# OpenVisualCloud/SVT-VP9

Measured on AMD Instinct MI355X. Metric: hot-path frames/sec (+ Mpixels/sec): block-level DSP path (picture analysis + ME + inter prediction from reconstructed references + DCT/quant/recon + deblock + reference padding), 3840x2160p60 yuv420p enc-mode 8; no mode decision, no entropy coding -- not encoded frames, higher is better.
Workload: dtype u8

## Files before the change

svt-vp9_amd/csrc/encdec.hip:

```cpp
#include <hip/hip_runtime.h>
#include <stdlib.h>
#include <string.h>
#include "svt_ctx.h"
#include "encdec_core.h"

#define ED_MAX_PICS 32
#define ED_MAX_SETS 8

struct svt_encdec_work {
    int           max_pics, width, height, n_sb, sb_cols, mi_rows, mi_cols;
    size_t        cap_per_pic;
    svt_tq_block *d_blocks;
    void         *last_hb;
    uint32_t     *d_pos;
    uint16_t     *d_eob;
    int32_t      *d_counts;
    int32_t      *d_totals, *d_bases;
    int32_t      *d_off_cnt;
    int32_t      *d_status;
    int32_t      *d_intra_sync;
    svt_quant_tables *d_qtabs;
    int16_t      *d_iscan;
    svt_encdec_stage_hook hook;
    void         *hook_user;
// ... 346 lines not shown
        if (svt_ctx_stage(ctx, sizeof qt, &h, &d)) return svt_set_error(SVT_HIP_ERR_NO_RESOURCES, "encdec: descriptor buffers");
        memcpy(h, qt, sizeof qt);
        HIP_TRY(hipMemcpyAsync(w->d_qtabs, h, sizeof qt, hipMemcpyHostToDevice, ctx->stream));
        svt_ctx_stage_commit(ctx);
    }
#define ED_STAGE(k) do { if (w->hook) w->hook(w->hook_user, (k)); } while (0)
    ED_STAGE(SVT_ENCDEC_STAGE_MC);
    int32_t rc = svt_hip_inter_pred_batch_device(ctx, n_pics, mcp);
    if (rc) return rc;
    ED_STAGE(SVT_ENCDEC_STAGE_LISTS);
    const int nwg = n_pics * hb.n_sb;
    hipLaunchKernelGGL(svt_tq_count_kernel, dim3(nwg), dim3(64), 0, ctx->stream, dB, w->d_counts, w->d_status);
    hipLaunchKernelGGL(svt_scan_sb_kernel, dim3(4 * n_pics), dim3(256), 0, ctx->stream, w->d_counts, hb.n_sb, w->d_totals);
    hipLaunchKernelGGL(svt_scan_pic_kernel, dim3(1), dim3(64), 0, ctx->stream, (const int32_t *)w->d_totals, n_pics, w->d_bases, w->d_off_cnt);
    hipLaunchKernelGGL(svt_tq_emit_kernel, dim3(nwg), dim3(64), 0, ctx->stream, dB, (const int32_t *)w->d_counts, (const int32_t *)w->d_bases, (svt_tq_block *)nullptr, w->d_pos);
    HIP_TRY(hipGetLastError());
    if (!w->last_hb) w->last_hb = malloc(sizeof hb);
    if (w->last_hb) memcpy(w->last_hb, &hb, sizeof hb);
    ED_STAGE(SVT_ENCDEC_STAGE_TQ);
    int32_t cap[4];
    for (int s = 0; s < 4; s++) cap[s] = (int32_t)((size_t)n_pics * width * height * 3 / 2 / (size_t)(16 << (2 * s)));
    rc = svt_tq_launch_device_lists(ctx, (const uint8_t *)src_lo, (const uint8_t *)pred_lo, recon_set, n_sets, nullptr, cap, w->d_off_cnt, w->d_qtabs, w->d_iscan,
                                    (int16_t *)q_lo, (int16_t *)dq_lo, w->d_eob, nullptr, w->d_pos, &dB->pic[0].g, (int)sizeof(ed_pic_dev), dB->iscan_off, hb.sb_cols);
    if (rc) return rc;
    ED_STAGE(SVT_ENCDEC_STAGE_SKIP);
    {
        const size_t map_bytes = (size_t)(width / 4) * (height / 4) * 3 / 2 * sizeof(uint16_t);
        uintptr_t    low = map_bytes;
        for (int i = 0; i < n_pics; i++) low |= (uintptr_t)pics[i].d_eob_map;
        if (!(low & 15))
            hipLaunchKernelGGL(svt_eob_map_clear_kernel, dim3(64, n_pics), dim3(256), 0, ctx->stream, dB, (int)(map_bytes / 16));
        else
            for (int i = 0; i < n_pics; i++) HIP_TRY(hipMemsetAsync(pics[i].d_eob_map, 0, map_bytes, ctx->stream));
    }
    for (int i = 0; i < n_pics; i++)
        if (pics[i].has_intra) {
            if (!flags->do_recon) return svt_set_error(SVT_HIP_ERR_BAD_PARAMETER, "encdec: intra blocks need the reconstruction (do_recon)");
            rc = svt_intra_launch(ctx, &pics[i], width, height, mi_stride, w->d_qtabs, w->d_iscan, hb.iscan_off, w->d_intra_sync, w->d_status, 1);
            if (rc) return rc;
        }
    {
        const int total_cap = (int)(w->cap_per_pic * (size_t)n_pics);
        int       g = (total_cap + 255) / 256;
        if (g > ctx->cu_count * 8) g = ctx->cu_count * 8;
        hipLaunchKernelGGL(svt_tq_skip_kernel, dim3(g), dim3(256), 0, ctx->stream, dB, (const int32_t *)w->d_off_cnt, (const uint32_t *)w->d_pos, (const uint16_t *)w->d_eob);
        hipLaunchKernelGGL(svt_skip_update_kernel, dim3((n_pics * hb.mi_rows * hb.mi_cols + 255) / 256), dim3(256), 0, ctx->stream, dB);
        HIP_TRY(hipGetLastError());
    }
    ED_STAGE(SVT_ENCDEC_STAGE_LF);
    if (flags->apply_loop_filter) {
        hipLaunchKernelGGL(svt_lf_mask_kernel, dim3(nwg), dim3(64), 0, ctx->stream, dB, w->d_status);
        HIP_TRY(hipGetLastError());
        rc = svt_hip_lf_batch_device(ctx, n_pics, rec, lfm, lfm_stride, thr, mi_rows_a, mi_cols_a, 0);
        if (rc) return rc;
    }
    ED_STAGE(SVT_ENCDEC_STAGE_PAD);
    if (flags->pad_reference && n_rec_pad) {
        rc = svt_hip_ref_pad_batch_device(ctx, n_rec_pad, rec_pad, pad_x, pad_y);
        if (rc) return rc;
    }
    ED_STAGE(SVT_ENCDEC_STAGE_END);
    return SVT_HIP_OK;
}

extern "C" int32_t svt_hip_encdec_intra_device(svt_hip_ctx *ctx, svt_encdec_work *w, const svt_encdec_picture *pic, int32_t width, int32_t height, int32_t mi_stride,
                                               int32_t q_index, const svt_encdec_flags *flags, const svt_lf_thresh *thr, int32_t pad_x, int32_t pad_y) {
    if (!ctx || !w || !pic || !flags || width != w->width || height != w->height || mi_stride < (width >> 3))
        return svt_set_error(SVT_HIP_ERR_BAD_PARAMETER, "encdec_intra: bad argument");
    if (!flags->do_recon) return svt_set_error(SVT_HIP_ERR_BAD_PARAMETER, "encdec_intra: intra prediction needs the reconstruction (do_recon)");
    if (flags->apply_loop_filter && !thr) return svt_set_error(SVT_HIP_ERR_BAD_PARAMETER, "encdec_intra: loop filter without thresholds");
    const svt_encdec_picture &p = *pic;
    if (!p.d_lf_mi || !p.src.y || !p.src.u || !p.src.v || !p.recon.y || !p.recon.u || !p.recon.v || !p.d_qcoeff || !p.d_eob_map || !p.d_nz ||
        (flags->apply_loop_filter && !p.d_lfm))
        return svt_set_error(SVT_HIP_ERR_BAD_PARAMETER, "encdec_intra: null picture field");
    if (((uintptr_t)p.d_qcoeff | (uintptr_t)p.d_dqcoeff) & 15) return svt_set_error(SVT_HIP_ERR_BAD_PARAMETER, "encdec_intra: coefficient arrays must be 16-byte aligned");
    if (p.recon.y_stride > 65535 || ((p.src.y_stride | p.src.uv_stride | p.recon.y_stride | p.recon.uv_stride) & 3) ||
        (((uintptr_t)p.src.y | (uintptr_t)p.src.u | (uintptr_t)p.src.v | (uintptr_t)p.recon.y | (uintptr_t)p.recon.u | (uintptr_t)p.recon.v) & 3) ||
        (p.pred.y && (((uintptr_t)p.pred.y | (uintptr_t)p.pred.u | (uintptr_t)p.pred.v | (uintptr_t)p.pred.y_stride | (uintptr_t)p.pred.uv_stride) & 3)))
        return svt_set_error(SVT_HIP_ERR_BAD_PARAMETER, "encdec_intra: planes and strides must be 4-byte aligned");
    if (p.pred.y && (!p.pred.u || !p.pred.v)) return svt_set_error(SVT_HIP_ERR_BAD_PARAMETER, "encdec_intra: prediction planes");
    HIP_TRY(hipSetDevice(ctx->device));
    ed_batch_dev hb;
    memset(&hb, 0, sizeof hb);
    fill_dims(hb, 1, width, height, mi_stride);
    const uint32_t *offs = nullptr;
    (void)svt_hip_vp9_iscan_tables(&offs, nullptr);
    hb.pic[0].lf_mi = p.d_lf_mi; hb.pic[0].nz = p.d_nz; hb.pic[0].eob_map = p.d_eob_map; hb.pic[0].lfm = p.d_lfm;
    const ed_batch_dev *dB = nullptr;
    if (stage_batch(ctx, hb, &dB)) return svt_set_error(SVT_HIP_ERR_NO_RESOURCES, "encdec_intra: descriptor buffers");
    {
        svt_quant_tables qt[2];
        if (svt_hip_quant_tables_for_qindex(q_index, qt) != SVT_HIP_OK) return svt_set_error(SVT_HIP_ERR_BAD_PARAMETER, "encdec_intra: q index");
        void *h = nullptr, *d = nullptr;
        if (svt_ctx_stage(ctx, sizeof qt, &h, &d)) return svt_set_error(SVT_HIP_ERR_NO_RESOURCES, "encdec_intra: descriptor buffers");
        memcpy(h, qt, sizeof qt);
        HIP_TRY(hipMemcpyAsync(w->d_qtabs, h, sizeof qt, hipMemcpyHostToDevice, ctx->stream));
        svt_ctx_stage_commit(ctx);
    }
    ED_STAGE(SVT_ENCDEC_STAGE_TQ);
    HIP_TRY(hipMemsetAsync(p.d_eob_map, 0, (size_t)(width / 4) * (height / 4) * 3 / 2 * sizeof(uint16_t), ctx->stream));
    HIP_TRY(hipMemsetAsync(p.d_nz, 0, (size_t)mi_stride * hb.mi_rows, ctx->stream));
    int32_t rc = svt_intra_launch(ctx, pic, width, height, mi_stride, w->d_qtabs, w->d_iscan, offs, w->d_intra_sync, w->d_status, 0);
    if (rc) return rc;
    ED_STAGE(SVT_ENCDEC_STAGE_SKIP);
    hipLaunchKernelGGL(svt_skip_update_kernel, dim3((hb.mi_rows * hb.mi_cols + 255) / 256), dim3(256), 0, ctx->stream, dB);
    HIP_TRY(hipGetLastError());
    ED_STAGE(SVT_ENCDEC_STAGE_LF);
    svt_yuv_planes rec = p.recon;
    rec.width = width; rec.height = height;
    if (flags->apply_loop_filter) {
        hipLaunchKernelGGL(svt_lf_mask_kernel, dim3(hb.n_sb), dim3(64), 0, ctx->stream, dB, w->d_status);
        HIP_TRY(hipGetLastError());
        const svt_lf_mask *lfm = p.d_lfm;
        const int32_t      lfm_stride = hb.sb_cols, mr = hb.mi_rows, mc = hb.mi_cols;
        rc = svt_hip_lf_batch_device(ctx, 1, &rec, &lfm, &lfm_stride, thr, &mr, &mc, 0);
        if (rc) return rc;
    }
    ED_STAGE(SVT_ENCDEC_STAGE_PAD);
    if (flags->pad_reference && !p.no_pad) {
        rc = svt_hip_ref_pad_batch_device(ctx, 1, &rec, pad_x, pad_y);
        if (rc) return rc;
    }
    ED_STAGE(SVT_ENCDEC_STAGE_END);
    return SVT_HIP_OK;
}

extern "C" int32_t svt_hip_md_intra_default_device(svt_hip_ctx *ctx, int32_t width, int32_t height, int32_t filter_level, svt_lf_mode_info *d_lf_mi, int32_t mi_stride) {
    if (!ctx || !d_lf_mi || width < 8 || height < 8 || (width & 7) || (height & 7) || mi_stride < (width >> 3))
        return svt_set_error(SVT_HIP_ERR_BAD_PARAMETER, "md_intra_default: bad argument");
    HIP_TRY(hipSetDevice(ctx->device));
    return svt_md_intra_default_launch(ctx, d_lf_mi, mi_stride, height >> 3, width >> 3, filter_level);
}

extern "C" void svt_hip_encdec_work_set_stage_hook(svt_encdec_work *w, svt_encdec_stage_hook hook, void *user) {
    if (!w) return;
    w->hook = hook;
    w->hook_user = user;
}

extern "C" int32_t svt_hip_encdec_work_status(svt_hip_ctx *ctx, svt_encdec_work *w, int32_t counts[8]) {
    if (!ctx || !w) return svt_set_error(SVT_HIP_ERR_BAD_PARAMETER, "encdec_status: null");
    HIP_TRY(hipSetDevice(ctx->device));
    int32_t h[9];
    HIP_TRY(hipMemcpyAsync(h, w->d_off_cnt, sizeof h, hipMemcpyDeviceToHost, ctx->stream));
    HIP_TRY(hipStreamSynchronize(ctx->stream));
    if (counts) memcpy(counts, h, 8 * sizeof(int32_t));
    if (h[8]) {
        HIP_TRY(hipMemsetAsync(w->d_status, 0, sizeof(int32_t), ctx->stream));
        return svt_set_error(SVT_HIP_ERR_BAD_PARAMETER, "encdec: malformed mode-info grid (block outside the picture, misaligned, or transform larger than its block)");
    }
    return SVT_HIP_OK;
}

extern "C" int32_t svt_hip_encdec_work_download(svt_hip_ctx *ctx, svt_encdec_work *w, svt_tq_block *blocks, uint32_t *pos, uint16_t *eob, int32_t capacity) {
    int32_t c[8];
    const int32_t rc = svt_hip_encdec_work_status(ctx, w, c);
    if (rc) return rc;
    const int32_t total = c[3] + c[7];
    if (total > capacity) return svt_set_error(SVT_HIP_ERR_NO_RESOURCES, "encdec_download: capacity");
    if (total > 0) {
        if (blocks) {
            if (!w->last_hb) return svt_set_error(SVT_HIP_ERR_BAD_PARAMETER, "encdec_download: no batch yet");
            if (!w->d_blocks && hipMalloc((void **)&w->d_blocks, w->cap_per_pic * (size_t)w->max_pics * sizeof(svt_tq_block)) != hipSuccess) {
                w->d_blocks = nullptr;
                return svt_set_error(SVT_HIP_ERR_NO_RESOURCES, "encdec_download: device memory");
            }
            const ed_batch_dev *dB = nullptr;
            if (stage_batch(ctx, *(const ed_batch_dev *)w->last_hb, &dB)) return svt_set_error(SVT_HIP_ERR_NO_RESOURCES, "encdec_download: descriptor buffers");
            hipLaunchKernelGGL(svt_tq_expand_kernel, dim3((total + 255) / 256), dim3(256), 0, ctx->stream, dB, (const int32_t *)w->d_off_cnt, (const uint32_t *)w->d_pos, w->d_blocks);
            HIP_TRY(hipGetLastError());
            HIP_TRY(hipMemcpyAsync(blocks, w->d_blocks, (size_t)total * sizeof(svt_tq_block), hipMemcpyDeviceToHost, ctx->stream));
        }
        if (pos) HIP_TRY(hipMemcpyAsync(pos, w->d_pos, (size_t)total * sizeof(uint32_t), hipMemcpyDeviceToHost, ctx->stream));
        if (eob) HIP_TRY(hipMemcpyAsync(eob, w->d_eob, (size_t)total * sizeof(uint16_t), hipMemcpyDeviceToHost, ctx->stream));
        HIP_TRY(hipStreamSynchronize(ctx->stream));
    }
    return total;
}

extern "C" int32_t svt_hip_md_default_batch_device(svt_hip_ctx *ctx, int32_t n_pics, const svt_me_pu_result *const *d_results, int32_t width, int32_t height,
                                                   uint32_t lambda, int32_t filter_level, svt_mc_mode_info *const *d_mc_mi, svt_lf_mode_info *const *d_lf_mi,
                                                   int32_t mi_stride) {
    if (!ctx || n_pics < 1 || !d_results || !d_mc_mi || !d_lf_mi || width < 8 || height < 8 || (width & 7) || (height & 7) || mi_stride < (width >> 3))
        return svt_set_error(SVT_HIP_ERR_BAD_PARAMETER, "md_default: bad argument");
    HIP_TRY(hipSetDevice(ctx->device));
    for (int first = 0; first < n_pics; first += ED_MAX_PICS) {
        const int n = n_pics - first < ED_MAX_PICS ? n_pics - first : ED_MAX_PICS;
        ed_batch_dev hb;
        memset(&hb, 0, sizeof hb);
        fill_dims(hb, n, width, height, mi_stride);
        hb.lambda = lambda; hb.filter_level = filter_level;
        for (int i = 0; i < n; i++) {
            if (!d_results[first + i] || !d_mc_mi[first + i] || !d_lf_mi[first + i]) return svt_set_error(SVT_HIP_ERR_BAD_PARAMETER, "md_default: null picture");
            hb.pic[i].res = d_results[first + i]; hb.pic[i].mc_mi = d_mc_mi[first + i]; hb.pic[i].lf_mi = d_lf_mi[first + i];
        }
        const ed_batch_dev *dB = nullptr;
        if (stage_batch(ctx, hb, &dB)) return svt_set_error(SVT_HIP_ERR_NO_RESOURCES, "md_default: descriptor buffers");
        hipLaunchKernelGGL(svt_md_default_kernel, dim3(n * hb.n_sb), dim3(64), 0, ctx->stream, dB);
        HIP_TRY(hipGetLastError());
    }
    return SVT_HIP_OK;
}

extern "C" int32_t svt_hip_lf_build_masks_device(svt_hip_ctx *ctx, int32_t n_pics, const svt_lf_mode_info *const *d_lf_mi, int32_t mi_stride, int32_t mi_rows,
                                                 int32_t mi_cols, svt_lf_mask *const *d_lfm) {
    if (!ctx || n_pics < 1 || !d_lf_mi || !d_lfm || mi_rows < 1 || mi_cols < 1 || mi_stride < mi_cols) return svt_set_error(SVT_HIP_ERR_BAD_PARAMETER, "lf_masks: bad argument");
    HIP_TRY(hipSetDevice(ctx->device));
    for (int first = 0; first < n_pics; first += ED_MAX_PICS) {
        const int n = n_pics - first < ED_MAX_PICS ? n_pics - first : ED_MAX_PICS;
        ed_batch_dev hb;
        memset(&hb, 0, sizeof hb);
        fill_dims(hb, n, mi_cols * 8, mi_rows * 8, mi_stride);
        for (int i = 0; i < n; i++) {
            if (!d_lf_mi[first + i] || !d_lfm[first + i]) return svt_set_error(SVT_HIP_ERR_BAD_PARAMETER, "lf_masks: null picture");
            hb.pic[i].lf_mi = (svt_lf_mode_info *)d_lf_mi[first + i]; hb.pic[i].lfm = d_lfm[first + i];
        }
        const ed_batch_dev *dB = nullptr;
        if (stage_batch(ctx, hb, &dB)) return svt_set_error(SVT_HIP_ERR_NO_RESOURCES, "lf_masks: descriptor buffers");
        hipLaunchKernelGGL(svt_lf_mask_kernel, dim3(n * hb.n_sb), dim3(64), 0, ctx->stream, dB, (int32_t *)nullptr);
        HIP_TRY(hipGetLastError());
    }
    return SVT_HIP_OK;
}
```

svt-vp9_amd/csrc/intra_kernel.hip:

```cpp
#include <hip/hip_runtime.h>
#include "tq_core.h"
#include "encdec_core.h"
#include "intra_pred.h"
#include <stdlib.h>

namespace {

struct intra_pic_dev {
    const uint8_t *src[3];
    uint8_t       *pred[3];
    uint8_t       *rec[3];
    int32_t        src_stride[2], pred_stride[2], rec_stride[2];
    const svt_lf_mode_info *mi;
    int32_t        mi_stride, mi_rows, mi_cols, sb_cols, sb_rows, width, height;
    const svt_quant_tables *qtabs;
    const int16_t *iscan;
    uint32_t       iscan_off[16];
    int16_t       *qcoeff, *dqcoeff;
    uint16_t      *eob_map;
    uint8_t       *nz;
    int32_t       *sync;
    int32_t       *status;
    int32_t        mixed;
};

#ifdef INTRA_FENCES
#define INTRA_WT false
#define INTRA_LD(p) (*(p))
#else
#define INTRA_WT true
#define INTRA_LD(p) __hip_atomic_load((p), __ATOMIC_RELAXED, __HIP_MEMORY_SCOPE_AGENT)
#endif
#ifdef INTRA_PROF
__device__ unsigned long long g_intra_fine[8];
#define IPF(k) do { if (lane == 0) { const unsigned long long n_ = __builtin_amdgcn_s_memtime(); atomicAdd(&g_intra_fine[k], n_ - ipf_t); ipf_t = n_; } } while (0)
#else
#define IPF(k) ((void)0)
#endif
template <int N>
__device__ __forceinline__ int intra_block(const intra_pic_dev &P, int plane, int x0, int y0, int mode, int sb, int32_t *tile, uint8_t *edge, int have_right = 0) {
    const int lane = (int)threadIdx.x, c = plane ? 1 : 0;
    const int rs = P.rec_stride[c];
    uint8_t  *rp = P.rec[plane];
    const int have_left = x0 > 0, have_top = y0 > 0;
    const bool active = lane < N;
    const int  i = lane % N;
#ifdef INTRA_PROF
    unsigned long long ipf_t = __builtin_amdgcn_s_memtime();
#endif
    uint32_t   srow[N / 4], prow[N / 4];
    constexpr uintptr_t AM = N >= 16 ? 15 : N - 1;
    {
        const uint8_t *sp = P.src[plane] + (size_t)(y0 + i) * P.src_stride[c] + x0;
        _Pragma("unroll") for (int q = 0; q < N / 4; q++) srow[q] = 0u;
        if (active) row_load<N>(sp, ((uintptr_t)sp & AM) == 0, srow);
    }
    {
        const int j = lane & 31;
        if (lane < 32) {
            if (j < N) edge[32 - (j + 1)] = have_left ? INTRA_LD(&rp[(size_t)(y0 + j) * rs + x0 - 1]) : (uint8_t)129;
        } else {
            if (j < N) {
                const uint8_t a = have_top ? INTRA_LD(&rp[(size_t)(y0 - 1) * rs + x0 + j]) : (uint8_t)127;
                edge[32 + 1 + j] = a;
                if (N == 4 && have_right) edge[32 + 1 + N + j] = have_top ? INTRA_LD(&rp[(size_t)(y0 - 1) * rs + x0 + N + j]) : (uint8_t)127;
                else if (j == N - 1) { _Pragma("unroll") for (int q = 0; q < N; q++) edge[32 + 1 + N + q] = a; }
            }
        }
        if (lane == 0) edge[32] = have_top ? (have_left ? INTRA_LD(&rp[(size_t)(y0 - 1) * rs + x0 - 1]) : (uint8_t)129) : (uint8_t)127;
    }
    __syncthreads();
    IPF(0);
    intra_pred_row<N>(edge, mode, i, have_left, have_top, prow);
    {
        if (active && P.pred[plane]) {
            uint8_t *pp = P.pred[plane] + (size_t)(y0 + i) * P.pred_stride[c] + x0;
            row_store<N>(pp, ((uintptr_t)pp & AM) == 0, prow);
        }
    }
    IPF(1);
    svt_tq_block k;
    k.src_off = k.pred_off = 0;
    k.recon_off = (uint32_t)y0 * (uint32_t)rs + (uint32_t)x0;
    k.coeff_off = (uint32_t)sb * SVT_SB_COEFFS + (plane == 0 ? 0u : plane == 1 ? 4096u : 5120u) + svt_zorder4((x0 & (plane ? 31 : 63)) >> 2, (y0 & (plane ? 31 : 63)) >> 2) * 16u;
    k.tx_size = (uint8_t)txcfg<N>::size;
    k.tx_type = (uint8_t)((plane == 0 && N < 32) ? intra_tx_type(mode) : 0);
    k.iscan_off = P.iscan_off[k.tx_size * 4 + k.tx_type];
    k.src_stride = k.pred_stride = 0; k.recon_stride = (uint16_t)rs;
    k.qtab = (uint8_t)c; k.do_recon = 1; k.partial32 = 0; k.pad_[0] = 0;
    const int pw4 = (plane ? P.width >> 1 : P.width) >> 2, w4 = P.width >> 2, h4 = P.height >> 2;
    const int eo = plane == 0 ? 0 : w4 * h4 + (plane == 2 ? (w4 >> 1) * (h4 >> 1) : 0);
    int32_t *t = tile + (lane / N) * (N * (N + 1));
    const int eob = tq_block_body<N, false, false, INTRA_WT>(k, active, i, t, srow, prow, P.qtabs, P.iscan, P.qcoeff, P.dqcoeff,
                                                   P.eob_map + eo + (y0 >> 2) * pw4 + (x0 >> 2), nullptr, nullptr, nullptr, nullptr, nullptr, rp);
    IPF(2);
    __builtin_amdgcn_fence(__ATOMIC_SEQ_CST, "workgroup");
    __syncthreads();
    IPF(3);
    return __builtin_amdgcn_readfirstlane(eob);
}

#ifndef INTRA_WAVES_PER_EU
#define INTRA_WAVES_PER_EU 4
#endif
#ifdef INTRA_NUM_VGPR
__attribute__((amdgpu_num_vgpr(INTRA_NUM_VGPR)))
#endif
__global__ __launch_bounds__(64) __attribute__((amdgpu_waves_per_eu(INTRA_WAVES_PER_EU, INTRA_WAVES_PER_EU))) void svt_intra_kernel(const intra_pic_dev P) {
    __shared__ int32_t tile[2 * 32 * 33];
    __shared__ uint8_t edge[128];
    __shared__ int32_t s_ticket;
    const int lane = (int)threadIdx.x, c_cols = (P.width + 15) >> 4, c_rows = (P.height + 15) >> 4, n_cell = c_cols * c_rows;
    const int n_diag = c_rows + c_cols - 1;
    __builtin_amdgcn_s_setprio(3);
#ifdef INTRA_PROF
  unsigned long long pf[5] = {0, 0, 0, 0, 0}, pf_n = 0;
#endif
  for (;;) {
    __syncthreads();
    if (lane == 0) s_ticket = atomicAdd(&P.sync[0], 1);
    __syncthreads();
#ifdef INTRA_PROF
    if (s_ticket >= 3 * n_cell) { if (lane == 0 && blockIdx.x == 0) printf("[intra-fine] refs %llu predict %llu tq %llu drain %llu (summed over all workgroups so far)\n", g_intra_fine[0], g_intra_fine[1], g_intra_fine[2], g_intra_fine[3]);
      if (lane == 0 && blockIdx.x < 2) printf("[intra-prof] wg %d cells %llu: ticket+map %llu wait %llu work %llu drain %llu publish %llu (100 MHz ticks)\n", (int)blockIdx.x, pf_n, pf[0], pf[1], pf[2], pf[3], pf[4]); break; }
    unsigned long long pt0 = __builtin_amdgcn_s_memtime();
#else
    if (s_ticket >= 3 * n_cell) break;
#endif
    const int ticket = s_ticket, plane = ticket % 3;
    const int n = ticket / 3, m = c_rows < c_cols ? c_rows : c_cols, M = c_rows < c_cols ? c_cols : c_rows;
    int lo = 0, hi = n_diag;
    auto count = [&](int d) -> int {
        const int a = d < m ? d : m;
        int       t = a * (a + 1) / 2;
        if (d > m) { const int fl = (d < M ? d : M) - m; t += fl * m; }
        if (d > M) { const int k = d - M; t += k * m - k * (k + 1) / 2; }
        return t;
    };
    while (hi - lo > 1) { const int mid = (lo + hi) >> 1; if (count(mid) <= n) lo = mid; else hi = mid; }
    const int d = lo, r_lo = d - (c_cols - 1) > 0 ? d - (c_cols - 1) : 0;
    const int cr = r_lo + (n - count(d)), cc = d - cr;
    const int cell = cr * c_cols + cc;
    int32_t  *done = P.sync + 2 + plane * n_cell;
    const int  br = cr & ~1, bc = cc & ~1;
    const int  ub_r = br * 2, ub_c = bc * 2;
    const svt_lf_mode_info b0 = P.mi[ub_r * P.mi_stride + ub_c];
    const bool big = b0.sb_type == 9 && !(b0.is_inter && P.mixed) && ub_r + 4 <= P.mi_rows && ub_c + 4 <= P.mi_cols;
    if (big && !(cr == br && cc == bc + 1)) continue;
    const int ur0 = cr * 2, uc0 = cc * 2;
#ifdef INTRA_PROF
    unsigned long long pt1 = __builtin_amdgcn_s_memtime();
#endif
    if (lane == 0) {
        const int wl_r = big ? br + 1 : cr, wl_c = (big ? bc : cc) - 1;
        const int wa_r = (big ? br : cr) - 1, wa_c = big ? bc + 1 : cc;
        if (wl_c >= 0) while (__hip_atomic_load(&done[wl_r * c_cols + wl_c], __ATOMIC_RELAXED, __HIP_MEMORY_SCOPE_AGENT) == 0) __builtin_amdgcn_s_sleep(2);
        if (wa_r >= 0) while (__hip_atomic_load(&done[wa_r * c_cols + wa_c], __ATOMIC_RELAXED, __HIP_MEMORY_SCOPE_AGENT) == 0) __builtin_amdgcn_s_sleep(2);
    }
    __syncthreads();
#ifdef INTRA_FENCES
    __builtin_amdgcn_fence(__ATOMIC_ACQUIRE, "agent");
#endif
#ifdef INTRA_PROF
    unsigned long long pt2 = __builtin_amdgcn_s_memtime();
#endif
    const int nu = big ? 1 : 4, u_r = big ? ub_r : ur0, u_c = big ? ub_c : uc0;
    for (int z = 0; z < nu; z++) {
        const int r = (z >> 1) & 1, c = z & 1;
        const int ur = u_r + r, uc = u_c + c;
        if (ur >= P.mi_rows || uc >= P.mi_cols) continue;
        const svt_lf_mode_info b = P.mi[ur * P.mi_stride + uc];
        const int sub = b.sb_type == 0;
        const int w8 = b.sb_type == 3 || sub ? 1 : b.sb_type == 6 ? 2 : b.sb_type == 9 ? 4 : 0;
        if (b.is_inter && P.mixed) continue;
        if (w8 == 0 || b.is_inter) { if (lane == 0) atomicOr(P.status, 1); continue; }
        if ((ur % w8) || (uc % w8)) continue;
        if (w8 == 4 && !big) { if (lane == 0) atomicOr(P.status, 1); continue; }
        const int mode = plane ? b.pad_[2] : b.pad_[1];
        if (ur + w8 > P.mi_rows || uc + w8 > P.mi_cols || b.tx_size != (sub ? 0 : w8 == 1 ? 1 : w8 == 2 ? 2 : 3) || (!sub && mode > 9) || b.pad_[2] > 9) {
            if (lane == 0) atomicOr(P.status, 1);
            continue;
        }
        const int sb = (ur >> 3) * P.sb_cols + (uc >> 3);
        const int x0 = plane ? uc * 4 : uc * 8, y0 = plane ? ur * 4 : ur * 8, nn = plane ? w8 * 4 : w8 * 8;
        int eob;
        if (sub && plane == 0) {
            const int m4 = (int)b.pad_[1] | (int)b.pad_[0] << 8;
            eob = 0;
            for (int q4 = 0; q4 < 4; q4++) {
                const int mq = (m4 >> (4 * q4)) & 15;
                if (mq > 9) { if (lane == 0) atomicOr(P.status, 1); continue; }
                eob |= intra_block<4>(P, 0, x0 + 4 * (q4 & 1), y0 + 4 * (q4 >> 1), mq, sb, tile, edge, !(q4 & 1));
            }
        }
        else if (nn == 32) eob = intra_block<32>(P, plane, x0, y0, mode, sb, tile, edge);
        else if (nn == 16) eob = intra_block<16>(P, plane, x0, y0, mode, sb, tile, edge);
        else if (nn == 8) eob = intra_block<8>(P, plane, x0, y0, mode, sb, tile, edge);
        else eob = intra_block<4>(P, plane, x0, y0, mode, sb, tile, edge);
        if (eob && lane == 0) P.nz[ur * P.mi_stride + uc] = 1;
    }
#ifdef INTRA_PROF
    unsigned long long pt3 = __builtin_amdgcn_s_memtime();
#endif
#ifdef INTRA_FENCES
    __builtin_amdgcn_fence(__ATOMIC_RELEASE, "agent");
    __syncthreads();
#else
    asm volatile("s_waitcnt vmcnt(0)" ::: "memory");
    __syncthreads();
#endif
#ifdef INTRA_PROF
    unsigned long long pt4 = __builtin_amdgcn_s_memtime();
#endif
    if (lane == 0) {
        if (big) {
            _Pragma("unroll") for (int k = 0; k < 4; k++) {
                const int rr = br + (k >> 1), c2 = bc + (k & 1);
                if (rr < c_rows && c2 < c_cols) __hip_atomic_store(&done[rr * c_cols + c2], 1, __ATOMIC_RELAXED, __HIP_MEMORY_SCOPE_AGENT);
            }
        } else __hip_atomic_store(&done[cell], 1, __ATOMIC_RELAXED, __HIP_MEMORY_SCOPE_AGENT);
    }
#ifdef INTRA_PROF
    { const unsigned long long pt5 = __builtin_amdgcn_s_memtime(); pf[0] += pt1 - pt0; pf[1] += pt2 - pt1; pf[2] += pt3 - pt2; pf[3] += pt4 - pt3; pf[4] += pt5 - pt4; pf_n++; }
#endif
  }
}

__global__ __launch_bounds__(256) void svt_md_intra_default_kernel(svt_lf_mode_info *mi, int mi_stride, int mi_rows, int mi_cols, int filter_level) {
    const int u = (int)(blockIdx.x * blockDim.x + threadIdx.x);
    if (u >= mi_rows * mi_cols) return;
    const int r = u / mi_cols, c = u % mi_cols;
    const int fit16 = (r & ~1) + 2 <= mi_rows && (c & ~1) + 2 <= mi_cols;
    svt_lf_mode_info m;
    m.sb_type = fit16 ? 6 : 3; m.tx_size = fit16 ? 2 : 1; m.skip = 0; m.is_inter = 0; m.filter_level = (uint8_t)filter_level;
    m.pad_[0] = m.pad_[1] = m.pad_[2] = 0;
    mi[r * mi_stride + c] = m;
}

}

int32_t svt_intra_launch(svt_hip_ctx *ctx, const svt_encdec_picture *p, int32_t width, int32_t height, int32_t mi_stride, const svt_quant_tables *d_qtabs,
                         const int16_t *d_iscan, const uint32_t iscan_off[16], int32_t *d_sync, int32_t *d_status, int32_t mixed) {
    intra_pic_dev P;
    memset(&P, 0, sizeof P);
    P.src[0] = p->src.y; P.src[1] = p->src.u; P.src[2] = p->src.v;
    P.pred[0] = p->pred.y; P.pred[1] = p->pred.u; P.pred[2] = p->pred.v;
    P.rec[0] = p->recon.y; P.rec[1] = p->recon.u; P.rec[2] = p->recon.v;
    P.src_stride[0] = p->src.y_stride; P.src_stride[1] = p->src.uv_stride;
    P.pred_stride[0] = p->pred.y_stride; P.pred_stride[1] = p->pred.uv_stride;
    P.rec_stride[0] = p->recon.y_stride; P.rec_stride[1] = p->recon.uv_stride;
    P.mi = p->d_lf_mi; P.mi_stride = mi_stride; P.mi_rows = height >> 3; P.mi_cols = width >> 3;
    P.sb_cols = (width + 63) >> 6; P.sb_rows = (height + 63) >> 6; P.width = width; P.height = height;
    P.qtabs = d_qtabs; P.iscan = d_iscan;
    for (int i = 0; i < 16; i++) P.iscan_off[i] = iscan_off[i];
    P.qcoeff = p->d_qcoeff; P.dqcoeff = p->d_dqcoeff; P.eob_map = p->d_eob_map; P.nz = p->d_nz; P.sync = d_sync; P.status = d_status; P.mixed = mixed;
    const int n_cell = ((width + 15) >> 4) * ((height + 15) >> 4);
    HIP_TRY(hipMemsetAsync(d_sync, 0, (size_t)(2 + 3 * n_cell) * sizeof(int32_t), ctx->stream));
    static const int wg_per_cu = [] { const char *e = getenv("SVT_HIP_INTRA_WG_PER_CU"); return e && atoi(e) > 0 ? atoi(e) : 2; }();
    static const int wg_cap = [] { const char *e = getenv("SVT_HIP_INTRA_WGS"); return e && atoi(e) > 0 ? atoi(e) : 0; }();
    int grid = ctx->cu_count * wg_per_cu;
    const int cap = ctx->intra_wgs > 0 ? ctx->intra_wgs : wg_cap;
    if (cap && grid > cap) grid = cap;
    if (grid > 3 * n_cell) grid = 3 * n_cell;
    hipLaunchKernelGGL(svt_intra_kernel, dim3(grid), dim3(64), 0, ctx->stream, P);
    HIP_TRY(hipGetLastError());
    return SVT_HIP_OK;
}

int32_t svt_md_intra_default_launch(svt_hip_ctx *ctx, svt_lf_mode_info *d_lf_mi, int32_t mi_stride, int32_t mi_rows, int32_t mi_cols, int32_t filter_level) {
    hipLaunchKernelGGL(svt_md_intra_default_kernel, dim3((mi_rows * mi_cols + 255) / 256), dim3(256), 0, ctx->stream, d_lf_mi, mi_stride, mi_rows, mi_cols, filter_level);
    HIP_TRY(hipGetLastError());
    return SVT_HIP_OK;
}
```

Before: 6349.

## Add specialized ≤16x16 intra kernel selected on device by mode-info scan

Adds a leaner intra reconstruction kernel for pictures whose blocks are all 16x16 or smaller. It caps VGPRs, uses a smaller LDS tile and a simplified per-block transform/quant/recon body. A new select kernel clears the sync buffer (replacing the memset) and scans the mode-info grid for 64x64 intra blocks. Its result makes either the specialized kernel or the general kernel run while the other exits immediately. This adds an extra launch per picture plus a serial single-block scan, in exchange for better occupancy and less work per cell in the common case.

```diff
diff --git a/svt-vp9_amd/csrc/encdec.hip b/svt-vp9_amd/csrc/encdec.hip
--- a/svt-vp9_amd/csrc/encdec.hip
+++ b/svt-vp9_amd/csrc/encdec.hip
@@ -522,6 +522,15 @@
     return SVT_HIP_OK;
 }
 
+extern "C" int32_t svt_hip_encdec_work_intra_instance(svt_hip_ctx *ctx, svt_encdec_work *w) {
+    if (!ctx || !w) return svt_set_error(SVT_HIP_ERR_BAD_PARAMETER, "encdec_intra_instance: null");
+    HIP_TRY(hipSetDevice(ctx->device));
+    int32_t h = -1;
+    HIP_TRY(hipMemcpyAsync(&h, w->d_intra_sync + 1, sizeof h, hipMemcpyDeviceToHost, ctx->stream));
+    HIP_TRY(hipStreamSynchronize(ctx->stream));
+    return h != 0;
+}
+
 extern "C" int32_t svt_hip_encdec_work_download(svt_hip_ctx *ctx, svt_encdec_work *w, svt_tq_block *blocks, uint32_t *pos, uint16_t *eob, int32_t capacity) {
     int32_t c[8];
     const int32_t rc = svt_hip_encdec_work_status(ctx, w, c);
diff --git a/svt-vp9_amd/csrc/intra_kernel.hip b/svt-vp9_amd/csrc/intra_kernel.hip
--- a/svt-vp9_amd/csrc/intra_kernel.hip
+++ b/svt-vp9_amd/csrc/intra_kernel.hip
@@ -3,6 +3,7 @@
 #include "encdec_core.h"
 #include "intra_pred.h"
 #include <stdlib.h>
+#include <string.h>
 
 namespace {
 
@@ -110,6 +111,7 @@
     __shared__ int32_t tile[2 * 32 * 33];
     __shared__ uint8_t edge[128];
     __shared__ int32_t s_ticket;
+    if (P.sync[1] == 0) return;
     const int lane = (int)threadIdx.x, c_cols = (P.width + 15) >> 4, c_rows = (P.height + 15) >> 4, n_cell = c_cols * c_rows;
     const int n_diag = c_rows + c_cols - 1;
     __builtin_amdgcn_s_setprio(3);
@@ -226,6 +228,310 @@
   }
 }
 
+
+template <int N>
+__device__ __forceinline__ int i16_tq_body(const svt_tq_block &k, const int tx_type, const bool active, const int i, int32_t *t, const uint32_t (&srow)[N / 4],
+                                           const uint32_t (&prow)[N / 4], const svt_quant_tables *__restrict__ qtabs, const int16_t *__restrict__ iscan_all,
+                                           int16_t *__restrict__ qcoeff, int16_t *__restrict__ dqcoeff, uint16_t *eob_slot, uint8_t *recon_base) {
+    static_assert(N <= 16, "the <= 16 instance");
+    constexpr int LS = N + 1;
+    const bool col_adst = tx_type == SVT_ADST_DCT || tx_type == SVT_ADST_ADST;
+    const bool row_adst = tx_type == SVT_DCT_ADST || tx_type == SVT_ADST_ADST;
+    int32_t v[N], o[N];
+    if (active) {
+        _Pragma("unroll") for (int cc = 0; cc < N; cc++)
+            t[i * LS + cc] = (int16_t)((int)((srow[cc >> 2] >> (8 * (cc & 3))) & 0xff) - (int)((prow[cc >> 2] >> (8 * (cc & 3))) & 0xff));
+    }
+    tq_block_sync();
+    _Pragma("unroll") for (int r = 0; r < N; r++) v[r] = t[r * LS + i];
+    if (tx_type == SVT_DCT_DCT) {
+        _Pragma("unroll") for (int r = 0; r < N; r++) v[r] *= (N == 4 ? 16 : 4);
+        if (N == 4 && i == 0 && v[0]) ++v[0];
+        fwd1d_dct<N>(v, o);
+        if (active) { _Pragma("unroll") for (int kk = 0; kk < N; kk++) t[kk * LS + i] = (int16_t)o[kk]; }
+    } else {
+        _Pragma("unroll") for (int r = 0; r < N; r++) v[r] = (int16_t)(v[r] * (N == 4 ? 16 : 4));
+        if (N == 4 && i == 0 && v[0]) v[0] = (int16_t)(v[0] + 1);
+        fwd1d_hybrid<N>(v, o, col_adst);
+        if (active) { _Pragma("unroll") for (int kk = 0; kk < N; kk++) t[kk * LS + i] = (N == 16) ? (int16_t)((o[kk] + 1 + (o[kk] < 0)) >> 2) : (int16_t)o[kk]; }
+    }
+    tq_block_sync();
+    _Pragma("unroll") for (int kk = 0; kk < N; kk++) v[kk] = t[i * LS + kk];
+    if (tx_type == SVT_DCT_DCT) {
+        if constexpr (N == 16) { _Pragma("unroll") for (int kk = 0; kk < N; kk++) v[kk] = (v[kk] + 1) >> 2; }
+        fwd1d_dct<N>(v, o);
+        _Pragma("unroll") for (int kk = 0; kk < N; kk++) {
+            if constexpr (N == 4) o[kk] = (int16_t)(((int16_t)o[kk] + 1) >> 2);
+            else if constexpr (N == 8) o[kk] = (int16_t)((int16_t)o[kk] / 2);
+            else o[kk] = (int16_t)o[kk];
+        }
+    } else {
+        fwd1d_hybrid<N>(v, o, row_adst);
+        _Pragma("unroll") for (int kk = 0; kk < N; kk++) {
+            const int32_t tt = o[kk];
+            o[kk] = (N == 4) ? (int16_t)((tt + 1) >> 2) : (N == 8) ? (int16_t)((tt + (tt < 0)) >> 1) : (int16_t)tt;
+        }
+    }
+    svt_quant_tables q;
+    {
+        const uint32_t *qp = (const uint32_t *)(qtabs + k.qtab);
+        uint32_t        qw5[5];
+        _Pragma("unroll") for (int j = 0; j < 5; j++) qw5[j] = qp[j];
+        q.zbin[0] = (int16_t)qw5[0]; q.zbin[1] = (int16_t)(qw5[0] >> 16); q.round[0] = (int16_t)qw5[1]; q.round[1] = (int16_t)(qw5[1] >> 16);
+        q.quant[0] = (int16_t)qw5[2]; q.quant[1] = (int16_t)(qw5[2] >> 16); q.quant_shift[0] = (int16_t)qw5[3]; q.quant_shift[1] = (int16_t)(qw5[3] >> 16);
+        q.dequant[0] = (int16_t)qw5[4]; q.dequant[1] = (int16_t)(qw5[4] >> 16);
+    }
+    const uint32_t *ip = (const uint32_t *)(iscan_all + k.iscan_off + i * N);
+    int eob = 0;
+    constexpr int VC = N == 4 ? 4 : 8;
+    uint32_t qw[VC / 2], dqw[VC / 2], isw = 0;
+    int16_t *qo = qcoeff + k.coeff_off + i * N, *dqo = dqcoeff + k.coeff_off + i * N;
+    _Pragma("unroll") for (int kk = 0; kk < N; kk++) {
+        if ((kk & 1) == 0) isw = ip[kk >> 1];
+        const int ac = (i | kk) != 0, cv = o[kk], sign = cv >> 31;
+        int       a = (cv ^ sign) - sign, level = 0, qv = 0, dv = 0;
+        if (a >= (ac ? q.zbin[1] : q.zbin[0])) {
+            const int tmp = clamp16(a + (ac ? q.round[1] : q.round[0]));
+            level = ((((tmp * (ac ? q.quant[1] : q.quant[0])) >> 16) + tmp) * (ac ? q.quant_shift[1] : q.quant_shift[0])) >> 16;
+            qv = (int16_t)((level ^ sign) - sign);
+            dv = (int16_t)(qv * (ac ? q.dequant[1] : q.dequant[0]));
+        }
+        if (active) t[i * LS + kk] = dv;
+        const int j = (kk % VC) >> 1;
+        if (kk & 1) { qw[j] |= (uint32_t)(uint16_t)qv << 16; dqw[j] |= (uint32_t)(uint16_t)dv << 16; }
+        else { qw[j] = (uint16_t)qv; dqw[j] = (uint16_t)dv; }
+        if ((kk % VC) == VC - 1 && active) {
+            if constexpr (N == 4) { *(uint2 *)qo = make_uint2(qw[0], qw[1]); if (dqcoeff) *(uint2 *)dqo = make_uint2(dqw[0], dqw[1]); }
+            else {
+                ((uint4 *)qo)[kk / VC] = make_uint4(qw[0], qw[1], qw[2], qw[3]);
+                if (dqcoeff) ((uint4 *)dqo)[kk / VC] = make_uint4(dqw[0], dqw[1], dqw[2], dqw[3]);
+            }
+        }
+        if (level && active) { const int pos = (int)((isw >> (16 * (kk & 1))) & 0xffff) + 1; eob = pos > eob ? pos : eob; }
+    }
+    eob = __builtin_amdgcn_readfirstlane(tq_lanes_max<N>(eob));
+    if (active && i == 0) *eob_slot = (uint16_t)eob;
+    const bool dct_path = tx_type == SVT_DCT_DCT;
+    bool dc_only = false;
+    int  nrows = N;
+    if (dct_path) {
+        if (N == 4) dc_only = eob <= 1;
+        else dc_only = eob == 1;
+        if (N == 8) nrows = eob <= 12 ? 4 : 8;
+        if (N == 16) nrows = eob <= 10 ? 4 : eob <= 38 ? 8 : 16;
+    }
+    uint32_t rw[N / 4];
+    tq_block_sync();
+    if (eob != 0 && !dc_only) {
+        if (i < nrows) {
+            _Pragma("unroll") for (int kk = 0; kk < N; kk++) v[kk] = t[i * LS + kk];
+            inv1d<N>(v, o, row_adst);
+        } else { _Pragma("unroll") for (int kk = 0; kk < N; kk++) o[kk] = 0; }
+        if (active) { _Pragma("unroll") for (int kk = 0; kk < N; kk++) t[i * LS + kk] = (int16_t)o[kk]; }
+        tq_block_sync();
+        _Pragma("unroll") for (int r = 0; r < N; r++) v[r] = t[r * LS + i];
+        inv1d<N>(v, o, col_adst);
+        tq_block_sync();
+        if (active) { _Pragma("unroll") for (int r = 0; r < N; r++) t[r * LS + i] = ((int16_t)o[r] + (1 << (txcfg<N>::shift - 1))) >> txcfg<N>::shift; }
+        tq_block_sync();
+        _Pragma("unroll") for (int q4 = 0; q4 < N / 4; q4++) {
+            uint32_t w = 0;
+            _Pragma("unroll") for (int b = 0; b < 4; b++) w |= (uint32_t)clip_add((int)((prow[q4] >> (8 * b)) & 0xff), t[i * LS + 4 * q4 + b]) << (8 * b);
+            rw[q4] = w;
+        }
+    } else {
+        int32_t a1 = 0;
+        if (eob != 0) {
+            int32_t d = tx_rsw((int16_t)t[0] * TX_C16);
+            d = tx_rsw(d * TX_C16);
+            a1 = (d + (1 << (txcfg<N>::shift - 1))) >> txcfg<N>::shift;
+        }
+        _Pragma("unroll") for (int q4 = 0; q4 < N / 4; q4++) {
+            uint32_t w = 0;
+            _Pragma("unroll") for (int b = 0; b < 4; b++) w |= (uint32_t)clip_add((int)((prow[q4] >> (8 * b)) & 0xff), a1) << (8 * b);
+            rw[q4] = w;
+        }
+    }
+    if (active) {
+        uint8_t *d = recon_base + k.recon_off + (size_t)i * k.recon_stride;
+        _Pragma("unroll") for (int q4 = 0; q4 < N / 4; q4++) __hip_atomic_store((uint32_t *)d + q4, rw[q4], __ATOMIC_RELAXED, __HIP_MEMORY_SCOPE_AGENT);
+    }
+    return eob;
+}
+
+template <int N>
+__device__ __noinline__ int i16_block(const intra_pic_dev &P, int plane, int x0, int y0, int mode, int sb, int32_t *tile, uint8_t *edge, int have_right = 0) {
+    mode = __builtin_amdgcn_readfirstlane(mode);
+    const int lane = (int)threadIdx.x, c = plane ? 1 : 0;
+    const int rs = P.rec_stride[c];
+    uint8_t  *rp = P.rec[plane];
+    const int have_left = x0 > 0, have_top = y0 > 0;
+    const bool active = lane < N;
+    const int  i = lane & (N - 1);
+    uint32_t   srow[N / 4], prow[N / 4];
+    constexpr uintptr_t AM = N >= 16 ? 15 : N - 1;
+    {
+        const uint8_t *sp = P.src[plane] + (size_t)(y0 + i) * P.src_stride[c] + x0;
+        _Pragma("unroll") for (int q = 0; q < N / 4; q++) srow[q] = 0u;
+        if (active) row_load<N>(sp, ((uintptr_t)sp & AM) == 0, srow);
+    }
+    {
+        const int j = lane & 31;
+        if (lane < 32) {
+            if (j < N) edge[32 - (j + 1)] = have_left ? INTRA_LD(&rp[(size_t)(y0 + j) * rs + x0 - 1]) : (uint8_t)129;
+        } else {
+            if (j < N) {
+                const uint8_t a = have_top ? INTRA_LD(&rp[(size_t)(y0 - 1) * rs + x0 + j]) : (uint8_t)127;
+                edge[32 + 1 + j] = a;
+                if (N == 4 && have_right) edge[32 + 1 + N + j] = have_top ? INTRA_LD(&rp[(size_t)(y0 - 1) * rs + x0 + N + j]) : (uint8_t)127;
+                else if (j == N - 1) { _Pragma("unroll") for (int q = 0; q < N; q++) edge[32 + 1 + N + q] = a; }
+            }
+        }
+        if (lane == 0) edge[32] = have_top ? (have_left ? INTRA_LD(&rp[(size_t)(y0 - 1) * rs + x0 - 1]) : (uint8_t)129) : (uint8_t)127;
+    }
+    __syncthreads();
+    intra_pred_row<N>(edge, mode, i, have_left, have_top, prow);
+    if (active && P.pred[plane]) {
+        uint8_t *pp = P.pred[plane] + (size_t)(y0 + i) * P.pred_stride[c] + x0;
+        row_store<N>(pp, ((uintptr_t)pp & AM) == 0, prow);
+    }
+    svt_tq_block k;
+    k.src_off = k.pred_off = 0;
+    k.recon_off = (uint32_t)y0 * (uint32_t)rs + (uint32_t)x0;
+    k.coeff_off = (uint32_t)sb * SVT_SB_COEFFS + (plane == 0 ? 0u : plane == 1 ? 4096u : 5120u) + svt_zorder4((x0 & (plane ? 31 : 63)) >> 2, (y0 & (plane ? 31 : 63)) >> 2) * 16u;
+    k.tx_size = (uint8_t)txcfg<N>::size;
+    const int tx_type = plane == 0 ? intra_tx_type(mode) : 0;
+    k.tx_type = (uint8_t)tx_type;
+    k.iscan_off = P.iscan_off[k.tx_size * 4 + tx_type];
+    k.src_stride = k.pred_stride = 0; k.recon_stride = (uint16_t)rs;
+    k.qtab = (uint8_t)c; k.do_recon = 1; k.partial32 = 0; k.pad_[0] = 0;
+    const int pw4 = (plane ? P.width >> 1 : P.width) >> 2, w4 = P.width >> 2, h4 = P.height >> 2;
+    const int eo = plane == 0 ? 0 : w4 * h4 + (plane == 2 ? (w4 >> 1) * (h4 >> 1) : 0);
+    const int eob = i16_tq_body<N>(k, tx_type, active, i, tile, srow, prow, P.qtabs, P.iscan, P.qcoeff, P.dqcoeff, P.eob_map + eo + (y0 >> 2) * pw4 + (x0 >> 2), rp);
+    __builtin_amdgcn_fence(__ATOMIC_SEQ_CST, "workgroup");
+    __syncthreads();
+    return eob;
+}
+
+__device__ __forceinline__ svt_lf_mode_info i16_mi(const svt_lf_mode_info *p) {
+    const uint2 w = *(const uint2 *)p;
+    const uint32_t a = __builtin_amdgcn_readfirstlane(w.x), b = __builtin_amdgcn_readfirstlane(w.y);
+    svt_lf_mode_info m;
+    m.sb_type = (uint8_t)a; m.tx_size = (uint8_t)(a >> 8); m.skip = (uint8_t)(a >> 16); m.is_inter = (uint8_t)(a >> 24);
+    m.filter_level = (uint8_t)b; m.pad_[0] = (uint8_t)(b >> 8); m.pad_[1] = (uint8_t)(b >> 16); m.pad_[2] = (uint8_t)(b >> 24);
+    return m;
+}
+
+__attribute__((amdgpu_num_vgpr(56))) __global__ __launch_bounds__(64) void svt_intra16_kernel(const intra_pic_dev P) {
+    if (P.sync[1] != 0) return;
+    const intra_pic_dev &PK = *(const intra_pic_dev *)__builtin_amdgcn_kernarg_segment_ptr();
+    if (PK.sync != P.sync || PK.status != P.status || PK.width != P.width || PK.mixed != P.mixed) {
+        if (threadIdx.x == 0) atomicOr(P.status, 1);
+        return;
+    }
+    __shared__ int32_t tile[16 * 17];
+    __shared__ uint8_t edge[128];
+    __shared__ int32_t s_ticket;
+    const int lane = (int)threadIdx.x, c_cols = (P.width + 15) >> 4, c_rows = (P.height + 15) >> 4, n_cell = c_cols * c_rows;
+    const int n_diag = c_rows + c_cols - 1;
+    __builtin_amdgcn_s_setprio(3);
+  for (;;) {
+    __syncthreads();
+    if (lane == 0) s_ticket = atomicAdd(&P.sync[0], 1);
+    __syncthreads();
+    const int ticket = __builtin_amdgcn_readfirstlane(s_ticket);
+    if (ticket >= 3 * n_cell) break;
+    const int plane = ticket % 3;
+    const int n = ticket / 3, m = c_rows < c_cols ? c_rows : c_cols, M = c_rows < c_cols ? c_cols : c_rows;
+    int lo = 0, hi = n_diag;
+    auto count = [&](int d) -> int {
+        const int a = d < m ? d : m;
+        int       t = a * (a + 1) / 2;
+        if (d > m) { const int fl = (d < M ? d : M) - m; t += fl * m; }
+        if (d > M) { const int k = d - M; t += k * m - k * (k + 1) / 2; }
+        return t;
+    };
+    while (hi - lo > 1) { const int mid = (lo + hi) >> 1; if (count(mid) <= n) lo = mid; else hi = mid; }
+    const int d = lo, r_lo = d - (c_cols - 1) > 0 ? d - (c_cols - 1) : 0;
+    const int cr = r_lo + (n - count(d)), cc = d - cr;
+    const int cell = cr * c_cols + cc;
+    int32_t  *done = P.sync + 2 + plane * n_cell;
+    if (lane == 0) {
+        if (cc > 0) while (__hip_atomic_load(&done[cr * c_cols + cc - 1], __ATOMIC_RELAXED, __HIP_MEMORY_SCOPE_AGENT) == 0) __builtin_amdgcn_s_sleep(2);
+        if (cr > 0) while (__hip_atomic_load(&done[(cr - 1) * c_cols + cc], __ATOMIC_RELAXED, __HIP_MEMORY_SCOPE_AGENT) == 0) __builtin_amdgcn_s_sleep(2);
+    }
+    __syncthreads();
+#ifdef INTRA_FENCES
+    __builtin_amdgcn_fence(__ATOMIC_ACQUIRE, "agent");
+#endif
+    const int u_r = cr * 2, u_c = cc * 2;
+    _Pragma("nounroll") for (int z = 0; z < 4; z++) {
+        const int ur = u_r + ((z >> 1) & 1), uc = u_c + (z & 1);
+        if (ur >= P.mi_rows || uc >= P.mi_cols) continue;
+        const svt_lf_mode_info b = i16_mi(&P.mi[ur * P.mi_stride + uc]);
+        const int sub = b.sb_type == 0;
+        const int w8 = b.sb_type == 3 || sub ? 1 : b.sb_type == 6 ? 2 : b.sb_type == 9 ? 4 : 0;
+        if (b.is_inter && P.mixed) continue;
+        if (w8 == 0 || b.is_inter) { if (lane == 0) atomicOr(P.status, 1); continue; }
+        if ((ur % w8) || (uc % w8)) continue;
+        if (w8 == 4) { if (lane == 0) atomicOr(P.status, 1); continue; }
+        const int mode = plane ? b.pad_[2] : b.pad_[1];
+        if (ur + w8 > P.mi_rows || uc + w8 > P.mi_cols || b.tx_size != (sub ? 0 : w8 == 1 ? 1 : 2) || (!sub && mode > 9) || b.pad_[2] > 9) {
+            if (lane == 0) atomicOr(P.status, 1);
+            continue;
+        }
+        const int sb = (ur >> 3) * P.sb_cols + (uc >> 3);
+        const int x0 = plane ? uc * 4 : uc * 8, y0 = plane ? ur * 4 : ur * 8, nn = plane ? w8 * 4 : w8 * 8;
+        int eob;
+        if (sub && plane == 0) {
+            const int m4 = (int)b.pad_[1] | (int)b.pad_[0] << 8;
+            eob = 0;
+            _Pragma("nounroll") for (int q4 = 0; q4 < 4; q4++) {
+                const int mq = (m4 >> (4 * q4)) & 15;
+                if (mq > 9) { if (lane == 0) atomicOr(P.status, 1); continue; }
+                eob |= i16_block<4>(PK, 0, x0 + 4 * (q4 & 1), y0 + 4 * (q4 >> 1), mq, sb, tile, edge, !(q4 & 1));
+            }
+        }
+        else if (nn == 16) eob = i16_block<16>(PK, plane, x0, y0, mode, sb, tile, edge);
+        else if (nn == 8) eob = i16_block<8>(PK, plane, x0, y0, mode, sb, tile, edge);
+        else eob = i16_block<4>(PK, plane, x0, y0, mode, sb, tile, edge);
+        if (eob && lane == 0) P.nz[ur * P.mi_stride + uc] = 1;
+    }
+#ifdef INTRA_FENCES
+    __builtin_amdgcn_fence(__ATOMIC_RELEASE, "agent");
+    __syncthreads();
+#else
+    asm volatile("s_waitcnt vmcnt(0)" ::: "memory");
+    __syncthreads();
+#endif
+    if (lane == 0) __hip_atomic_store(&done[cell], 1, __ATOMIC_RELAXED, __HIP_MEMORY_SCOPE_AGENT);
+  }
+}
+
+__global__ __launch_bounds__(256) void svt_intra_select_kernel(int32_t *sync, int n_sync, const svt_lf_mode_info *mi, int mi_stride, int mi_rows, int mi_cols,
+                                                               int mixed, int force) {
+    for (int x = (int)(blockIdx.x * blockDim.x + threadIdx.x); x < n_sync; x += (int)(gridDim.x * blockDim.x))
+        if (x != 1) sync[x] = 0;
+    if (blockIdx.x != 0) return;
+    const int r4 = (mi_rows + 3) >> 2, c4 = (mi_cols + 3) >> 2, n = r4 * c4;
+    int any = force == 1;
+    if (!force)
+        for (int u0 = (int)threadIdx.x; u0 < n; u0 += 8 * (int)blockDim.x) {
+            uint8_t st[8], in[8];
+            _Pragma("unroll") for (int k = 0; k < 8; k++) {
+                const int u = u0 + k * (int)blockDim.x;
+                st[k] = in[k] = 0;
+                if (u < n) {
+                    const svt_lf_mode_info *b = &mi[(u / c4) * 4 * mi_stride + (u % c4) * 4];
+                    st[k] = b->sb_type; in[k] = b->is_inter;
+                }
+            }
+            _Pragma("unroll") for (int k = 0; k < 8; k++) any |= st[k] == 9 && !(in[k] && mixed);
+        }
+    any = __syncthreads_or(any);
+    if (threadIdx.x == 0) sync[1] = any;
+}
+
 __global__ __launch_bounds__(256) void svt_md_intra_default_kernel(svt_lf_mode_info *mi, int mi_stride, int mi_rows, int mi_cols, int filter_level) {
     const int u = (int)(blockIdx.x * blockDim.x + threadIdx.x);
     if (u >= mi_rows * mi_cols) return;
@@ -255,13 +561,17 @@
     for (int i = 0; i < 16; i++) P.iscan_off[i] = iscan_off[i];
     P.qcoeff = p->d_qcoeff; P.dqcoeff = p->d_dqcoeff; P.eob_map = p->d_eob_map; P.nz = p->d_nz; P.sync = d_sync; P.status = d_status; P.mixed = mixed;
     const int n_cell = ((width + 15) >> 4) * ((height + 15) >> 4);
-    HIP_TRY(hipMemsetAsync(d_sync, 0, (size_t)(2 + 3 * n_cell) * sizeof(int32_t), ctx->stream));
+    const char *inst = getenv("SVT_HIP_INTRA_INSTANCE");
+    const int   force = !inst ? 0 : !strcmp(inst, "general") ? 1 : !strcmp(inst, "le16") ? 2 : 0;
+    const int   n_sync = 2 + 3 * n_cell;
+    hipLaunchKernelGGL(svt_intra_select_kernel, dim3((n_sync + 1023) / 1024), dim3(256), 0, ctx->stream, d_sync, n_sync, p->d_lf_mi, mi_stride, P.mi_rows, P.mi_cols, mixed, force);
     static const int wg_per_cu = [] { const char *e = getenv("SVT_HIP_INTRA_WG_PER_CU"); return e && atoi(e) > 0 ? atoi(e) : 2; }();
     static const int wg_cap = [] { const char *e = getenv("SVT_HIP_INTRA_WGS"); return e && atoi(e) > 0 ? atoi(e) : 0; }();
     int grid = ctx->cu_count * wg_per_cu;
     const int cap = ctx->intra_wgs > 0 ? ctx->intra_wgs : wg_cap;
     if (cap && grid > cap) grid = cap;
     if (grid > 3 * n_cell) grid = 3 * n_cell;
+    hipLaunchKernelGGL(svt_intra16_kernel, dim3(grid), dim3(64), 0, ctx->stream, P);
     hipLaunchKernelGGL(svt_intra_kernel, dim3(grid), dim3(64), 0, ctx->stream, P);
     HIP_TRY(hipGetLastError());
     return SVT_HIP_OK;
```

After: 6424, median of 6. 1.01x the previous value.
